# QWERTY6191/projected-lmc

Measured on AMD Instinct MI355X. Metric: MLL+grad iters/sec, n=8192 16-task LMC, higher is better.
Workload: dtype f32; 1 GPU; C3: ProjectedGPModel+ProjectedLMCmll exact training step (PLMC_fast), n=8192 d=8 p=16 q=8 Matern-5/2 fp32; latents sharded q/N per GPU; n_points=8192, n_dim=8, n_tasks=16, n_latents=8, parallelism=latent-shard x1

## Files before the change

### projected-lmc_amd/csrc/api.hip

```cpp
#include <stdlib.h>
#include <mutex>
#include <vector>

#include "api_common.hpp"
#include "../../include/plmc.h"

namespace plmc {
char *err_buf() {
  static thread_local char buf[256] = {0};
  return buf;
}

static const char *kProfNames[PK_COUNT] = {"k_assemble", "k_write_rhs", "k_assemble_cross", "k_diag",   "k_panel",
                                           "k_trail",    "k_wdiag",     "k_trtri_row",      "k_extract_col",
                                           "k_wt_matvec", "k_kinv_grad", "k_reduce_grad", "k_kernel_vjp",
                                           "sweep_total", "k_trail_row", "k_trail_head", "k_gpanel", "k_split_w", "k_posterior_moments", "k_trmm_ut"};
struct ProfRec { int id; hipEvent_t a, b; double flops, bytes; };
static unsigned g_prof_mask = 0;
static std::vector<ProfRec> g_recs;
static std::vector<hipEvent_t> g_free;

static hipEvent_t get_event() {
  if (!g_free.empty()) { hipEvent_t e = g_free.back(); g_free.pop_back(); return e; }
  hipEvent_t e;
  if (hipEventCreate(&e) != hipSuccess) return nullptr;
  return e;
}

static std::recursive_mutex g_api_mutex;
void api_lock() { g_api_mutex.lock(); }
void api_unlock() { g_api_mutex.unlock(); }

static Knobs g_knobs;
static bool g_knobs_loaded = false;
static void load_knobs() {
  const char *h = getenv("PLMC_HALF_TILES"), *g = getenv("PLMC_GRP");
  g_knobs.half_tiles = h ? (atoi(h) == 1 ? 1e30 : (double)atoi(h)) : 640.0;
  g_knobs.grp = g ? atoi(g) : 0;
  g_knobs.serial = getenv("PLMC_SERIAL") && atoi(getenv("PLMC_SERIAL")) != 0;
  g_knobs.bulk_lds = getenv("PLMC_BULK_LDS") ? atoi(getenv("PLMC_BULK_LDS")) : -1;
  g_knobs.split = getenv("PLMC_SPLIT") ? atoi(getenv("PLMC_SPLIT")) : 2;
  if (g_knobs.split != 0 && g_knobs.split != 3) g_knobs.split = 2;
  g_knobs.bulk_streams = getenv("PLMC_BULK_STREAMS") ? atoi(getenv("PLMC_BULK_STREAMS")) : 2;
  g_knobs.chain = getenv("PLMC_CHAIN") ? atoi(getenv("PLMC_CHAIN")) : 1;
  g_knobs.chain_nw = getenv("PLMC_CHAIN_NW") ? atoi(getenv("PLMC_CHAIN_NW")) : 0;
  g_knobs.chain_edge = getenv("PLMC_CHAIN_EDGE") ? atoi(getenv("PLMC_CHAIN_EDGE")) : 0;
  g_knobs_loaded = true;
}
const Knobs &knobs() {
  if (!g_knobs_loaded) {
    std::lock_guard<std::recursive_mutex> lk(g_api_mutex);
    if (!g_knobs_loaded) load_knobs();
  }
  return g_knobs;
}

constexpr int SWEEP_CTX = 2;
struct SweepCtx {
  hipStream_t caller = nullptr;
  bool used = false;
  unsigned long long stamp = 0;
  hipStream_t side[2] = {nullptr, nullptr};
  hipEvent_t ev[16] = {nullptr};
};
static SweepCtx g_ctx[64][SWEEP_CTX];
static unsigned long long g_stamp = 0;
static thread_local int t_ctx = 0;
static SweepCtx *cur_ctx() {
  int dev = 0;
  if (hipGetDevice(&dev) != hipSuccess || dev < 0 || dev >= 64) return nullptr;
  return &g_ctx[dev][t_ctx];
}
hipStream_t side_stream(int which) {
  SweepCtx *c = cur_ctx();
  if (!c || which < 0 || which > 1) return nullptr;
  if (!c->side[which]) {
    int lo = 0, hi = 0;
    (void)hipDeviceGetStreamPriorityRange(&lo, &hi);
    if (hipStreamCreateWithPriority(&c->side[which], hipStreamNonBlocking, hi) != hipSuccess) c->side[which] = nullptr;
  }
  return c->side[which];
}
hipEvent_t sync_event(int idx) {
  SweepCtx *c = cur_ctx();
  if (!c) return nullptr;
  hipEvent_t &e = c->ev[idx & 15];
  if (!e && hipEventCreateWithFlags(&e, hipEventDisableTiming) != hipSuccess) e = nullptr;
  return e;
}
void bind_sweep_ctx(hipStream_t caller, int e_prev_idx) {
  int dev = 0;
  if (hipGetDevice(&dev) != hipSuccess || dev < 0 || dev >= 64) { t_ctx = 0; return; }
  SweepCtx *set = g_ctx[dev];
  int pick = -1;
  for (int i = 0; i < SWEEP_CTX; ++i)
    if (set[i].used && set[i].caller == caller) pick = i;
  if (pick < 0) {
    for (int i = 0; i < SWEEP_CTX && pick < 0; ++i)
      if (!set[i].used) pick = i;
    if (pick < 0) {
      pick = 0;
      for (int i = 1; i < SWEEP_CTX; ++i)
        if (set[i].stamp < set[pick].stamp) pick = i;
      if (set[pick].ev[e_prev_idx & 15]) (void)hipStreamWaitEvent(caller, set[pick].ev[e_prev_idx & 15], 0);
    }
    set[pick].caller = caller;
    set[pick].used = true;
  }
  set[pick].stamp = ++g_stamp;
  t_ctx = pick;
}

template <typename T>
__global__ __launch_bounds__(NTHREADS) void k_mfma_rate(T *sink, int iters) {
  using Tr = Traits<T>;
  typename Tr::acc_t acc[16];
#pragma unroll
  for (int i = 0; i < 16; ++i)
#pragma unroll
    for (int r = 0; r < 4; ++r) acc[i][r] = T(0);
  T a[4], b[4];
#pragma unroll
  for (int i = 0; i < 4; ++i) { a[i] = T(1) + T(threadIdx.x & 7) * T(1e-3) + T(i); b[i] = T(0.5) - T(i) * T(1e-3); }
#pragma unroll 1
  for (int it = 0; it < iters; ++it) {
#pragma unroll
    for (int i = 0; i < 16; ++i) acc[i] = Tr::mfma(a[i >> 2], b[i & 3], acc[i]);
  }
  T s = T(0);
#pragma unroll
  for (int i = 0; i < 16; ++i) s += acc[i][0] + acc[i][1] + acc[i][2] + acc[i][3];
  sink[(size_t)blockIdx.x * NTHREADS + threadIdx.x] = s;
}

typedef __bf16 rate_bf16x8 __attribute__((ext_vector_type(8)));
__global__ __launch_bounds__(NTHREADS) void k_mfma_rate_bf16(float *sink, int iters) {
  f32x4 acc[16];
#pragma unroll
  for (int i = 0; i < 16; ++i)
#pragma unroll
    for (int r = 0; r < 4; ++r) acc[i][r] = 0.f;
  rate_bf16x8 a[4], b[4];
#pragma unroll
  for (int i = 0; i < 4; ++i)
#pragma unroll
    for (int j = 0; j < 8; ++j) { a[i][j] = (__bf16)(1.0f + 0.01f * (float)((threadIdx.x + j) & 7) + (float)i); b[i][j] = (__bf16)(0.5f - 0.01f * (float)(i + j)); }
#pragma unroll 1
  for (int it = 0; it < iters; ++it) {
#pragma unroll
    for (int i = 0; i < 16; ++i) acc[i] = __builtin_amdgcn_mfma_f32_16x16x32_bf16(a[i >> 2], b[i & 3], acc[i], 0, 0, 0);
  }
  float s = 0.f;
#pragma unroll
  for (int i = 0; i < 16; ++i) s += acc[i][0] + acc[i][1] + acc[i][2] + acc[i][3];
  sink[(size_t)blockIdx.x * NTHREADS + threadIdx.x] = s;
}

template <typename T, bool BF16 = false> static int mfma_rate_impl(void *sink, int64_t sink_bytes, double *tflops) {
  int dev = 0;
  hipDeviceProp_t prop;
  if (hipGetDevice(&dev) != hipSuccess || hipGetDeviceProperties(&prop, dev) != hipSuccess) return fail("plmc_prof_mfma_rate", "no device");
  const int grid = 4 * prop.multiProcessorCount, iters = 4000;
  if (!sink || !tflops || sink_bytes < (int64_t)grid * NTHREADS * (int64_t)sizeof(T)) return fail("plmc_prof_mfma_rate", "sink too small");
  hipEvent_t e0 = nullptr, e1 = nullptr;
  if (hipEventCreate(&e0) != hipSuccess || hipEventCreate(&e1) != hipSuccess) return fail("plmc_prof_mfma_rate", "event");
  double best = 0.0;
  for (int rep = 0; rep < 3; ++rep) {
    (void)hipEventRecord(e0, nullptr);
    if (BF16) hipLaunchKernelGGL(k_mfma_rate_bf16, dim3(grid), dim3(NTHREADS), 0, nullptr, (float *)sink, iters);
    else hipLaunchKernelGGL(k_mfma_rate<T>, dim3(grid), dim3(NTHREADS), 0, nullptr, (T *)sink, iters);
    (void)hipEventRecord(e1, nullptr);
    float ms = 0.f;
    if (hipEventSynchronize(e1) != hipSuccess || hipEventElapsedTime(&ms, e0, e1) != hipSuccess) break;
    const double fl = (double)grid * (NTHREADS / 64) * (double)iters * 16.0 * 2.0 * 16 * 16 * (BF16 ? 32 : 4);
    if (ms > 0.f && fl / (ms * 1e-3) / 1e12 > best) best = fl / (ms * 1e-3) / 1e12;
  }
  (void)hipEventDestroy(e0);
  (void)hipEventDestroy(e1);
  *tflops = best;
  return launch_status("plmc_prof_mfma_rate");
}

ProfScope::ProfScope(int id, hipStream_t st, double flops, double bytes) : idx_(-1), st_(st) {
  api_lock();
  if (!((g_prof_mask >> id) & 1u) || g_recs.size() >= (1u << 20)) return;
  ProfRec r{id, get_event(), get_event(), flops, bytes};
  if (!r.a || !r.b) return;
  (void)hipEventRecord(r.a, st);
  g_recs.push_back(r);
  idx_ = (long)g_recs.size() - 1;
}
ProfScope::~ProfScope() {
  if (idx_ >= 0) (void)hipEventRecord(g_recs[idx_].b, st_);
  api_unlock();
}
}

extern "C" {
// ... 40 lines not shown
```

### projected-lmc_amd/csrc/api_common.hpp

```cpp
#pragma once
#include <hip/hip_runtime.h>
#include <stdint.h>
#include <stdio.h>
#include <string.h>

#include "gemm_core.hpp"
#include "covariance.hpp"

namespace plmc {

constexpr int MAX_DIM = 32;
constexpr int MAX_COMP = 4;
constexpr int SM_MAX_MIX = 8;
constexpr int SM_MAX_DIM = 8;
constexpr int PER_MAX_DIM = 8;
constexpr int RQ_MAX_DIM = 16;
constexpr int LPER_MAX_DIM = 8;
constexpr int DOT_MAX_DIM = 16;
constexpr int DOT_MAX_POWER = 8;
constexpr int SUM_MAX_DIM = 8;
constexpr int FAM_PUBLIC_BASE = 16;
enum { F_PER = 5, F_RQ = 6, F_LPER = 7 };

char *err_buf();

inline int fail(const char *fn, const char *msg) {
  snprintf(err_buf(), 256, "%s: %s", fn, msg);
  return -1;
}

inline int launch_status(const char *fn) {
  hipError_t e = hipGetLastError();
  if (e != hipSuccess) {
    snprintf(err_buf(), 256, "%s: HIP launch failed: %s", fn, hipGetErrorString(e));
    return -2;
  }
  return 0;
}

#define PLMC_REQUIRE(cond, msg) \
  do { if (!(cond)) return plmc::fail(__func__, msg); } while (0)

enum ProfKernel { PK_ASSEMBLE, PK_WRITE_RHS, PK_CROSS, PK_DIAG, PK_PANEL, PK_TRAIL, PK_WDIAG, PK_TRTRI, PK_EXTRACT,
                  PK_WTMV, PK_KINV_GRAD, PK_REDUCE, PK_VJP, PK_SWEEP, PK_TRAIL_ROW, PK_TRAIL_HEAD, PK_GPANEL, PK_SPLIT, PK_POST, PK_TRMM, PK_COUNT };

struct ProfScope {
  ProfScope(int id, hipStream_t st, double flops, double bytes);
  ~ProfScope();
  long idx_;
  hipStream_t st_;
};

struct Knobs {
  double half_tiles;
  int grp;
  bool serial;
  int bulk_lds;
  int split;
  int bulk_streams;
  int chain;
  int chain_edge;
  int chain_nw;
};
const Knobs &knobs();

enum CovFamily { COV_PLAIN, COV_ADD, COV_SM, COV_PER, COV_RQ, COV_LPER, COV_SUM, COV_DOT };
struct CovTable {
  CovFamily family;
  int kind, d, ncomp;
  const void *ell, *second, *oscale;
  const void *third = nullptr;
  int fams = 0;
  bool of_sum = false;
  static CovTable plain(int kind, int d, const void *ell, const void *oscale) { return {COV_PLAIN, kind, d, 1, ell, nullptr, oscale}; }
  static CovTable add(int kind, int d, int ncomp, const void *ell, const void *oscale) { return {COV_ADD, kind, d, ncomp, ell, nullptr, oscale}; }
  static CovTable sm(int d, int nmix, const void *scales, const void *means, const void *weights) { return {COV_SM, 0, d, nmix, scales, means, weights}; }
  static CovTable per(int d, const void *ell, const void *period, const void *oscale) { return {COV_PER, 0, d, 1, ell, period, oscale}; }
  static CovTable rq(int d, const void *ell, const void *alpha, const void *oscale) { return {COV_RQ, 0, d, 1, ell, alpha, oscale}; }
  static CovTable lper(int d, const void *ell, const void *period, const void *rbf_ell, const void *oscale) {
    return {COV_LPER, 0, d, 1, ell, period, oscale, rbf_ell};
  }
  static CovTable dot(int d, int power, const void *v, const void *c, const void *oscale) { return {COV_DOT, 0, d, power, v, c, oscale}; }
  int power() const { return ncomp; }
  static CovTable sum(int d, int ncomp, const int *fam, const void *table, const void *oscale) {
    CovTable t{COV_SUM, 0, d, ncomp, table, nullptr, oscale};
    if (!fam) t.fams = -3;
    if (!fam || ncomp < 1 || ncomp > MAX_COMP) return t;
    for (int g = 0; g < ncomp; ++g) {
      const int f = fam[g];
      int code;
      if (f >= K_RBF && f <= K_MATERN52) code = f;
      else if (f >= FAM_PUBLIC_BASE && f <= FAM_PUBLIC_BASE + 2) code = F_PER + (f - FAM_PUBLIC_BASE);
      else { t.fams = f == K_SPLINE ? -2 : -1; return t; }
      t.fams |= code << (4 * g);
    }
    return t;
  }
  int fam_of(int g) const { return (fams >> (4 * g)) & 15; }
  CovTable member(const void *ell_, const void *period_, const void *rbf_, const void *alpha_, const void *os_) const {
    const int f = fam_of(0);
    CovTable t = f == F_PER ? per(d, ell_, period_, os_) : f == F_RQ ? rq(d, ell_, alpha_, os_) : f == F_LPER ? lper(d, ell_, period_, rbf_, os_)
                                                                                                          : plain(f, d, ell_, os_);
    t.of_sum = true;
    return t;
  }
  template <typename T> CovTable member_of_latent(int lat) const {
    const T *rec = (const T *)ell + (int64_t)lat * (3 * d + 1);
    return member(rec, rec + d, rec + 2 * d, rec + 3 * d, oscale ? (const T *)oscale + lat : nullptr);
  }
  bool single_member() const { return family == COV_SUM && ncomp == 1; }
  const char *check() const {
    if (family == COV_SUM) {
      if (ncomp < 1 || ncomp > MAX_COMP) return "need 1 <= components <= plmc_sum_max_components()";
      if (d <= 0 || d > SUM_MAX_DIM) return "need 0 < d <= plmc_sum_max_dim()";
      if (fams == -3 || !ell) return "null pointer";
      if (fams == -2) return "the spline kernel is not a member of a sum (members: the stationary kinds 0..3, PLMC_FAM_PERIODIC, PLMC_FAM_RQ, PLMC_FAM_LPER)";
      if (fams < 0) return "unknown member family code (members: the stationary kinds 0..3, PLMC_FAM_PERIODIC, PLMC_FAM_RQ, PLMC_FAM_LPER; no spectral mixture)";
      return nullptr;
    }
    if (family == COV_ADD) {
      if (kind < 0 || kind > K_MATERN52) return "additive kernels take the stationary kinds only (no spline kernel)";
      if (ncomp < 1 || ncomp > MAX_COMP) return "need 1 <= components <= plmc_max_components()";
    } else if (family == COV_SM) {
      if (ncomp < 1 || ncomp > SM_MAX_MIX) return "need 1 <= mixtures <= plmc_sm_max_mixtures()";
      if (d <= 0 || d > SM_MAX_DIM) return "need 0 < d <= plmc_sm_max_dim()";
    } else if (family == COV_PER) {
      if (d <= 0 || d > PER_MAX_DIM) return "need 0 < d <= plmc_per_max_dim()";
    } else if (family == COV_RQ) {
      if (d <= 0 || d > RQ_MAX_DIM) return "need 0 < d <= plmc_rq_max_dim()";
    } else if (family == COV_LPER) {
      if (d <= 0 || d > LPER_MAX_DIM) return "need 0 < d <= plmc_lper_max_dim()";
      if (!third) return "null pointer";
    } else if (family == COV_DOT) {
      if (d <= 0 || d > DOT_MAX_DIM) return "need 0 < d <= plmc_dot_max_dim()";
      if (ncomp < 1 || ncomp > DOT_MAX_POWER) return "need 1 <= power <= plmc_dot_max_power()";
    }
    return (family == COV_SM || family == COV_PER || family == COV_RQ || family == COV_LPER || family == COV_DOT) && !second ? "null pointer" : nullptr;
  }
  CovFamily route() const { return family == COV_ADD && ncomp == 1 ? COV_PLAIN : family; }
  int partials_rows() const { return family == COV_ADD || family == COV_SM || family == COV_SUM ? ncomp : 1; }
};
#define PLMC_REQUIRE_TABLE(t) \
  do { if (const char *why_ = (t).check()) return plmc::fail(__func__, why_); } while (0)

struct AssembleJob {
  CovTable table;
  int n;
  const void *X, *noise;
};
int assemble_rows(const AssembleJob &job, int elem_bytes, void *A, int64_t lda, int64_t strideA, int q, int ib0, int nrows, void *stream,
                  int ncols = -1, int skip = 0);

hipStream_t side_stream(int which = 0);
hipEvent_t sync_event(int idx);
void bind_sweep_ctx(hipStream_t caller, int e_prev_idx);

inline bool aligned16(const void *p) { return (reinterpret_cast<uintptr_t>(p) & 15) == 0; }

}
```

### projected-lmc_amd/csrc/potrf.hip

```cpp
#include <stdlib.h>
#include "api_common.hpp"
#include "covariance.hpp"
#include "diag_block.hpp"
#include "bf3_engine.hpp"
#include "chain_engine.hpp"
#include "vd_layout.hpp"
#include "../../include/plmc.h"

namespace plmc {

template <typename T> constexpr int CHAIN_BURST = sizeof(T) == 8 ? 4 : 8;

template <typename T> struct ColMap {
  int u0, nU, Taug, w0, nW;
  int64_t n_pad;
  T *W;
  int64_t ldw, strideW;
};

template <typename T, int NT, bool BURSTED = false>
__global__ __launch_bounds__(NTHREADS, TILE_MIN_WAVES<T>) void k_panel(T *A, int64_t lda, int64_t strideA, int r, ColMap<T> cm,
                                                     const T *__restrict__ Vd, int64_t strideV) {
  __builtin_amdgcn_s_setprio(3);
  __shared__ __align__(16) T smem[tile_smem_elems<T>()];
// ... 513 lines not shown
  else if (t < cm.nU + cm.Taug) { colp = cm.n_pad + (int64_t)(t - cm.nU) * NB; D = A + (int64_t)lat * strideA + (int64_t)g0 * NB * lda + colp; }
  else {
    ldd = cm.ldw;
    colp = wcol0 + (int64_t)(cm.w0 + t - cm.nU - cm.Taug) * NB;
    D = cm.W + (int64_t)lat * cm.strideW + (int64_t)g0 * NB * ldd + (int64_t)(cm.w0 + t - cm.nU - cm.Taug) * NB;
  }
  const int nm = (G + 1) / 2;
  const unsigned short *Vp = VgP + (int64_t)lat * vgp_lat_stride, *Rp = Praw + (int64_t)lat * praw_lat_stride + colp * 8;
  unsigned short *Pp = Pl + (int64_t)lat * pl_lat_stride + colp * 8;
  int64_t pld = lda;
  if (fam == 1) { Pp = Wk + (int64_t)lat * wk_lat_stride + b3_index<S>((int64_t)g0 * NB, 0, colp - wcol0, cm.n_pad); pld = cm.n_pad; }
  const int half = __builtin_amdgcn_readfirstlane((int)threadIdx.x >> 8), tid = (int)threadIdx.x & 255;
#pragma unroll 1
  for (int pass = 0; pass < 2; ++pass) {
    const int a = pass == 0 ? nm - 1 - y : ((paired && y < nm - 1 - y) ? y : -1);
    if (a < 0) break;
    const int i0 = 2 * a, rows = G - i0 < 2 ? G - i0 : 2;
    Acc<float> acc0, acc1;
    acc0.zero();
    acc1.zero();
    b3_mainloop<S>(acc0, acc1, Vp + (int64_t)i0 * NB * 8, (int64_t)GMAX * NB, Rp, lda, (i0 + rows) * NB, lds);
    b3_combine<S>(acc0, acc1, unscale);
    const int i = i0 + half;
    b3_writeback<S, WB_STORE, true>(acc0, D + (int64_t)i * NB * ldd, ldd, reinterpret_cast<float *>(lds + half * B3_WB_BYTES), tid, half < rows,
                                    Pp + (int64_t)i * 16 * S::NPL * pld * 8, pld, true, pscale);
    __syncthreads();
  }
}

template <typename T>
__global__ __launch_bounds__(NTHREADS) void k_extract_col(const T *__restrict__ A, int64_t n_pad, int64_t lda,
                                                           int64_t strideA, int c, T *__restrict__ z,
                                                           double *__restrict__ quad) {
  __shared__ double red[NTHREADS];
  const int lat = blockIdx.x;
  const T *Al = A + (int64_t)lat * strideA + n_pad + c;
  double s = 0.0;
  for (int64_t i = threadIdx.x; i < n_pad; i += NTHREADS) {
    T v = Al[i * lda];
    z[(int64_t)lat * n_pad + i] = v;
    s += (double)v * (double)v;
  }
  red[threadIdx.x] = s;
  __syncthreads();
  for (int o = NTHREADS / 2; o > 0; o >>= 1) {
    if (threadIdx.x < o) red[threadIdx.x] += red[threadIdx.x + o];
    __syncthreads();
  }
  if (threadIdx.x == 0) quad[lat] = red[0];
}

constexpr int WTMV_NT = 1024;
template <typename T, int CW = NB>
__global__ __launch_bounds__(WTMV_NT * CW / NB) void k_wt_matvec(const T *__restrict__ W, int64_t n_pad, int64_t ldw,
                                                                 int64_t strideW, const T *__restrict__ z,
                                                                 T *__restrict__ alpha) {
  using vec_t = typename Traits<T>::vec_t;
  constexpr int EPV = Traits<T>::EPV;
  constexpr int LPR = CW / EPV;
  constexpr int NRG = WTMV_NT / (NB / EPV);
  __shared__ double red[NRG][CW];
  const int lat = blockIdx.y;
  const int cl = (threadIdx.x % LPR) * EPV, rg = threadIdx.x / LPR;
  const int64_t colw = (int64_t)blockIdx.x * CW;
  const int64_t col0 = colw / NB * NB;
  const T *Wl = W + (int64_t)lat * strideW + colw + cl;
  const T *zl = z + (int64_t)lat * n_pad;
  double s[EPV];
#pragma unroll
  for (int e = 0; e < EPV; ++e) s[e] = 0.0;
  constexpr int U = CW == NB ? 4 : 8;
  for (int64_t l = col0 + rg; l < n_pad; l += U * NRG) {
    vec_t v[U];
    T zz[U];
#pragma unroll
    for (int u = 0; u < U; ++u) {
      const int64_t ll = l + u * NRG;
      const int64_t lc = ll < n_pad ? ll : n_pad - 1;
      v[u] = *reinterpret_cast<const vec_t *>(Wl + lc * ldw);
      const T zv = zl[lc];
      zz[u] = ll < n_pad ? zv : T(0);
    }
#pragma unroll
    for (int u = 0; u < U; ++u)
#pragma unroll
      for (int e = 0; e < EPV; ++e) s[e] += (double)v[u][e] * (double)zz[u];
  }
#pragma unroll
  for (int e = 0; e < EPV; ++e) red[rg][cl + e] = s[e];
  __syncthreads();
  if (threadIdx.x < CW) {
    double t = 0.0;
#pragma unroll
    for (int g = 0; g < NRG; ++g) t += red[g][threadIdx.x];
    alpha[(int64_t)lat * n_pad + colw + threadIdx.x] = (T)t;
  }
}

template <typename T>
__global__ __launch_bounds__(WTMV_NT) void k_w_diag(const T *__restrict__ W, int64_t n_pad, int64_t ldw, int64_t strideW,
                                                    T *__restrict__ kd) {
  using vec_t = typename Traits<T>::vec_t;
  constexpr int EPV = Traits<T>::EPV;
  constexpr int LPR = 128 / EPV;
  constexpr int NRG = WTMV_NT / LPR;
  __shared__ double red[NRG][NB];
  const int lat = blockIdx.y;
  const int cl = (threadIdx.x % LPR) * EPV, rg = threadIdx.x / LPR;
  const int64_t col0 = (int64_t)blockIdx.x * NB;
  const T *Wl = W + (int64_t)lat * strideW + col0 + cl;
  double s[EPV];
#pragma unroll
  for (int e = 0; e < EPV; ++e) s[e] = 0.0;
  for (int64_t l = col0 + rg; l < n_pad; l += 4 * NRG) {
    vec_t v[4];
#pragma unroll
    for (int u = 0; u < 4; ++u) {
      const int64_t ll = l + u * NRG;
      v[u] = *reinterpret_cast<const vec_t *>(Wl + (ll < n_pad ? ll : n_pad - 1) * ldw);
    }
#pragma unroll
    for (int u = 0; u < 4; ++u)
      if (l + u * NRG < n_pad) {
#pragma unroll
        for (int e = 0; e < EPV; ++e) s[e] += (double)v[u][e] * (double)v[u][e];
      }
  }
#pragma unroll
  for (int e = 0; e < EPV; ++e) red[rg][cl + e] = s[e];
  __syncthreads();
  if (threadIdx.x < NB) {
    double t = 0.0;
#pragma unroll
    for (int g = 0; g < NRG; ++g) t += red[g][threadIdx.x];
    kd[(int64_t)lat * n_pad + col0 + threadIdx.x] = (T)t;
  }
}

template <typename T, class S>
struct Sweep {
  static constexpr bool bf3 = !std::is_void<S>::value;
  static_assert(!bf3 || sizeof(T) == 4, "split schemes stand in for fp32 products");
  static constexpr double nb = NB, nb3 = nb * nb * nb, esz = sizeof(T);

  T *A;
  int64_t n_pad, lda, strideA, naug_pad, wcol0;
  int q, m, Taug;
  bool with_inverse, keep;
  const float *eig_lo = nullptr;
  double *logdet = nullptr;
  int *info = nullptr;
  T *Vd, *Wg, *Vg2[2], *Ph, *Pbulk;
  unsigned short *Pl[2], *Praw, *VgP2[2], *Wk, *Uk;
  float *scl;
  int64_t strideV, pl_lat, sc_lat, uk_step;
  T *WA;
  const Knobs &kn;
  double hthr;
  unsigned bulk_lds;
  int grp, ng, chain_pool;
  hipStream_t st, C = nullptr, H = nullptr;
  hipEvent_t e_entry = nullptr, e_v = nullptr, e_gh = nullptr, e_p = nullptr, e_hd = nullptr, e_tail = nullptr, e_doneC = nullptr,
             e_doneH = nullptr, e_prev = nullptr, e_sc = nullptr;

  Sweep(T *A_, int64_t n_pad_, int64_t lda_, int naug, int64_t wcol0_, int64_t strideA_, T *Vd_, int q_, bool with_inverse_, bool keep_,
        int grp_, unsigned bulk_lds_, hipStream_t st_)
      : A(A_), n_pad(n_pad_), lda(lda_), strideA(strideA_), naug_pad(plmc_pad(naug)), wcol0(wcol0_), q(q_), m((int)(n_pad_ / NB)),
        Taug((int)(plmc_pad(naug) / NB)), with_inverse(with_inverse_), keep(keep_), Vd(Vd_), kn(knobs()), hthr(kn.half_tiles),
        bulk_lds(bulk_lds_), grp(grp_), st(st_) {
    const VdLayout L(n_pad, lda, (int)sizeof(T), keep);
    strideV = L.stride();
    pl_lat = L.stride_u16();
    sc_lat = L.stride_f32();
    Wg = L.at<T>(Vd, L.wg);
    Ph = L.at<T>(Vd, L.ph);
    Pbulk = L.at<T>(Vd, L.pbulk);
    for (int b = 0; b < 2; ++b) {
      Vg2[b] = L.at<T>(Vd, L.vg[b]);
      Pl[b] = bf3 ? L.at<unsigned short>(Vd, L.pl[b]) : nullptr;
      VgP2[b] = bf3 ? L.at<unsigned short>(Vd, L.vgp[b]) : nullptr;
    }
    Praw = bf3 ? L.at<unsigned short>(Vd, L.praw) : nullptr;
    scl = bf3 ? L.at<float>(Vd, L.scl) : nullptr;
    Wk = (bf3 && with_inverse) ? L.at<unsigned short>(Vd, L.wk) : nullptr;
    Uk = keep ? L.at<unsigned short>(Vd, L.uk) : nullptr;
    uk_step = L.plane_blocks * NB * NB * 2;
    WA = with_inverse ? A + wcol0 : nullptr;
    ng = (m + grp - 1) / grp;
    chain_pool = kn.chain_nw > 0 ? (kn.chain_nw < 200 ? kn.chain_nw : 200) : (q >= 8 ? 80 : (q >= 4 ? 44 : (q >= 2 ? 36 : 31)));
  }

  int G0(int gi) const { return gi < ng ? gi * grp : m; }
  ColMap<T> cm_tri(int g0, int u0, int nU, int w0, int nW) const {
    return ColMap<T>{u0, nU, 0, w0, nW, n_pad, Wg - (int64_t)g0 * NB * LDG - (int64_t)g0 * NB, (int64_t)LDG, strideV};
  }
  ColMap<T> cm_buf(int u0, int nU, int taug, int w0, int nW) const { return ColMap<T>{u0, nU, taug, w0, WA ? nW : 0, n_pad, WA, lda, strideA}; }
  unsigned short *planes(int g0) const { return keep ? Uk + (int64_t)(g0 / grp) * uk_step : Pl[(g0 / grp) & 1]; }

  void clear() {
    hipLaunchKernelGGL(k_zero_diag_out<T>, dim3(m > GMAX ? m : GMAX, q), dim3(NTHREADS), 0, st, Vd, strideV, m, Wg, (int64_t)LDG,
                       strideV, (int64_t)NB * LDG + NB, GMAX, VdLayout::CTR);
  }
  void diag(int r, int g0, hipStream_t s) {
    ProfScope ps(PK_DIAG, s, q * (2.0 / 3.0) * nb3, q * 3.0 * nb * nb * esz);
    T *wout = Wg + (int64_t)(r - g0) * NB * LDG + (int64_t)(r - g0) * NB;
    hipLaunchKernelGGL((k_diag<T>), dim3(q), dim3(DIAG_NT), 0, s, A, lda, strideA, r, Vd, strideV, wout, (int64_t)LDG, strideV);
  }
  void panel(int r, const ColMap<T> &cm, hipStream_t s) {
    const int nt = cm.nU + cm.Taug + cm.nW;
    if (nt == 0) return;
    ProfScope ps(PK_PANEL, s, q * (double)nt * nb3, q * 2.0 * nt * nb * nb * esz);
    if ((double)nt * q <= hthr && q <= 2)
      hipLaunchKernelGGL((k_panel<T, 2, true>), dim3(nt, q, 2), dim3(NTHREADS), 0, s, A, lda, strideA, r, cm, Vd, strideV);
    else if ((double)nt * q <= hthr)
      hipLaunchKernelGGL((k_panel<T, 2>), dim3(nt, q, 2), dim3(NTHREADS), 0, s, A, lda, strideA, r, cm, Vd, strideV);
    else
      hipLaunchKernelGGL((k_panel<T, 4>), dim3(nt, q, 1), dim3(NTHREADS), 0, s, A, lda, strideA, r, cm, Vd, strideV);
  }
  void update(int ib0, int nrows, int r_lo, int r_hi, const ColMap<T> &cm, hipStream_t s, int cls, int skip_ib = 0, int skip_jb = 0,
              bool crit = false, int raw_end = 0) {
    const int Cn = cm.nU + cm.Taug + cm.nW;
    if (nrows <= 0 || Cn == 0) return;
    const double depth = (r_hi - r_lo + 1) * nb, nr = (double)nrows;
    double tilesU = 0.0, halfU = 0.0;
    for (int i = 0; i < nrows; ++i)
      for (int t = 0; t < cm.nU; ++t) {
        const int ib = ib0 + i, jb = cm.u0 + t;
        if (jb < ib || (ib < skip_ib && jb < skip_jb)) continue;
        tilesU += 1.0;
        if (jb == ib) halfU += 0.5;
      }
    double depthW = 0.0;
    int nfirst = 0;
    for (int c = 0; c < cm.nW; ++c) {
      const int cb = cm.w0 + c;
      depthW += (cb >= r_lo ? (r_hi - cb + 1) : (r_hi - r_lo + 1)) * nb;
      nfirst += cb >= r_lo;
    }
    const double flops = 2.0 * nb * nb * (depth * (tilesU - halfU) + nr * (depth * cm.Taug + depthW));
    const double bytes = (2.0 * (tilesU + nr * (cm.Taug + cm.nW)) - nr * nfirst) * nb * nb * esz;
    ProfScope ps(cls, s, q * flops, q * bytes);
    if constexpr (bf3) {
      if (cls == PK_TRAIL || cls == PK_TRAIL_HEAD) {
        const dim3 grid(Cn, (nrows + 1) / 2, q);
        const unsigned short *pl = planes(r_lo);
#define PLMC_UPD3(ROLE)                                                                                                                    \
  hipLaunchKernelGGL((k_update_bf3<S, ROLE>), grid, dim3(B3_NT), 0, s, A, lda, strideA, ib0, nrows, r_lo, r_hi, cm, skip_ib, skip_jb, pl, \
                     pl_lat, wcol0, Praw, pl_lat, raw_end, (const float *)scl, sc_lat, Wk, pl_lat)
        if (cls == PK_TRAIL) PLMC_UPD3(0);
        else if (crit) PLMC_UPD3(2);
        else PLMC_UPD3(3);
#undef PLMC_UPD3
        return;
      }
    }
    const bool half = cls != PK_TRAIL && (double)Cn * nrows * q <= hthr;
    const unsigned dyn = (cls == PK_TRAIL || (cls == PK_TRAIL_HEAD && !crit)) ? bulk_lds : 0u;
    const dim3 grid(Cn, half ? 2 * nrows : nrows, q);
#define PLMC_UPD(ROLE, MT) \
  hipLaunchKernelGGL((k_update<T, ROLE, MT>), grid, dim3(NTHREADS), dyn, s, A, lda, strideA, ib0, r_lo, r_hi, cm, skip_ib, skip_jb)
    if (cls == PK_TRAIL_ROW) { if (half && q <= 2 && r_hi == r_lo) PLMC_UPD(4, 2); else if (half) PLMC_UPD(1, 2); else PLMC_UPD(1, 4); }
    else if (cls == PK_TRAIL_HEAD && crit) { if (half) PLMC_UPD(2, 2); else PLMC_UPD(2, 4); }
    else if (cls == PK_TRAIL_HEAD) { if (half) PLMC_UPD(3, 2); else PLMC_UPD(3, 4); }
    else PLMC_UPD(0, 4);
#undef PLMC_UPD
  }
  void gpanel(int g0, int G, const ColMap<T> &cm, int buf, hipStream_t s, int head) {
    const int nt = cm.nU + cm.Taug + cm.nW;
    if (nt == 0) return;
    const double prods = G * (G + 1) / 2.0;
    ProfScope ps(PK_GPANEL, s, q * (double)nt * prods * 2.0 * nb3, q * (double)nt * (prods + G) * nb * nb * esz);
    if constexpr (bf3) {
      const int nm = (G + 1) / 2;
      hipLaunchKernelGGL((k_gpanel_bf3<S>), dim3(nt, head ? nm : (nm + 1) / 2, q), dim3(B3_NT), 0, s, A, lda, strideA, g0, G, cm,
                         (const unsigned short *)VgP2[buf], pl_lat, (const unsigned short *)Praw, pl_lat, planes(g0), pl_lat, wcol0,
                         (const float *)scl, sc_lat, head ? 0 : 1, Wk, pl_lat);
    } else {
      T *Pb = head ? Ph : Pbulk;
      const int64_t ldp = head ? (int64_t)LDG : lda;
      if (head)
        hipLaunchKernelGGL((k_gpanel_rows<T, 1>), dim3(nt, 2 * G, q), dim3(NTHREADS), 0, s, (const T *)A, lda, strideA, g0, G, cm,
                           (const T *)Vg2[buf], (int64_t)LDG, strideV, Pb, ldp, strideV);
      else
        hipLaunchKernelGGL((k_gpanel_rows<T, 0>), dim3(nt, (G + 1) / 2, q), dim3(NTHREADS), bulk_lds, s, (const T *)A, lda, strideA, g0, G, cm,
                           (const T *)Vg2[buf], (int64_t)LDG, strideV, Pb, ldp, strideV);
      hipLaunchKernelGGL((k_gpanel_copy<T>), dim3(nt, G, q), dim3(NTHREADS), 0, s, A, lda, strideA, g0, cm, (const T *)Pb, ldp, strideV);
    }
  }
  void scan(hipStream_t s, int64_t row0, int64_t row1, int part0, int parts) {
    if constexpr (bf3) {
      if (S::NPL == 2)
        hipLaunchKernelGGL(k_scale_scan, dim3(parts, q), dim3(NTHREADS), 0, s, (const float *)A, n_pad, row0, row1, lda, strideA, (int)naug_pad, scl,
                           sc_lat, part0);
    }
  }
  void split_scales(hipStream_t s) {
    if constexpr (bf3) hipLaunchKernelGGL((k_split_scales<S>), dim3(q), dim3(64), 0, s, n_pad, eig_lo, scl, sc_lat);
  }
  int finish(hipStream_t s) {
    hipLaunchKernelGGL(k_logdet<T>, dim3(q), dim3(NTHREADS), 0, s, (const T *)A, n_pad, lda, strideA, logdet, info,
                       (const T *)(Wg + VdLayout::CTL), strideV, q);
    return launch_status("potrf_impl");
  }

  static constexpr int CHAIN_QB = 32;
  void chain(int gi, hipStream_t s) {
    const int g0 = G0(gi), g1 = G0(gi + 1);
    if (kn.chain) {
      const int G = g1 - g0;
      ProfScope ps(PK_DIAG, s, q * (2.0 / 3.0) * nb3 * G, q * 3.0 * nb * nb * esz * G);
      const bool edge = gi == 0 || gi + 2 >= ng;
      const int pool = (edge && kn.chain_edge > 0) ? kn.chain_edge : chain_pool;
      for (int l0 = 0; l0 < q; l0 += CHAIN_QB) {
        const int ql = q - l0 < CHAIN_QB ? q - l0 : CHAIN_QB;
        hipLaunchKernelGGL((k_chain<T>), dim3(ql + (G > 1 ? pool : 0)), dim3(CH_NT), 0, s, A + (int64_t)l0 * strideA, lda, strideA, g0, G,
                           Vd + (int64_t)l0 * strideV, strideV, Wg + (int64_t)l0 * strideV, strideV, ql);
      }
      return;
    }
    for (int r = g0; r < g1; ++r) {
      diag(r, g0, s);
      panel(r, cm_tri(g0, r + 1, g1 - 1 - r, g0, r - g0), s);
      if (r + 1 < g1) update(r + 1, g1 - r - 1, r, r, cm_tri(g0, r + 1, g1 - r - 1, g0, r + 1 - g0), s, PK_TRAIL_ROW);
    }
  }
  void vtrans(int gi, hipStream_t s, bool from_w = false) {
    const int g0 = G0(gi), G = G0(gi + 1) - g0;
    T *const tri = WA ? WA + (int64_t)g0 * NB * lda + (int64_t)g0 * NB : (T *)nullptr;
    hipLaunchKernelGGL((k_vtrans<T, S>), dim3(bf3 ? GMAX * GMAX : G * (G + 1) / 2, q), dim3(NTHREADS), 0, s, from_w ? (const T *)tri : (const T *)Wg,
                       from_w ? lda : (int64_t)LDG, from_w ? strideA : strideV, strideV, Vg2[gi & 1], G, from_w ? (T *)nullptr : tri, lda, strideA,
                       VgP2[gi & 1], pl_lat, (const float *)scl, sc_lat);
  }
  void wtri_planes(int gi, hipStream_t s) {
    if constexpr (bf3) {
      if (!WA) return;
      const int g0 = G0(gi), G = G0(gi + 1) - g0;
      hipLaunchKernelGGL((k_wtri_planes<S>), dim3(G * (G + 1) / 2, q), dim3(NTHREADS), 0, s, (const float *)WA, lda, strideA, g0, (const float *)scl,
                         sc_lat, Wk, pl_lat, n_pad);
    }
  }
  void raw_planes0(hipStream_t s, const ColMap<T> &cm) {
    if constexpr (bf3) {
      const int nt = cm.nU + cm.Taug + cm.nW;
      if (nt > 0)
        hipLaunchKernelGGL((k_raw_planes<S>), dim3(nt, G0(1), q), dim3(NTHREADS), 0, s, (const float *)A, lda, strideA, 0, cm, Praw, pl_lat, wcol0,
                           (const float *)scl, sc_lat);
    }
  }

  bool bind_streams() {
    if (!kn.serial) bind_sweep_ctx(st, 8);
    C = kn.serial ? nullptr : side_stream();
    H = kn.serial ? nullptr : (kn.bulk_streams == 1 ? st : side_stream(1));
    hipEvent_t *const ev[] = {&e_entry, &e_v, &e_gh, &e_p, &e_hd, &e_tail, &e_doneC, &e_doneH, &e_prev};
    bool la = C && H && ng > 2;
    for (int i = 0; i < 9; ++i) la = (*ev[i] = sync_event(i)) && la;
    e_sc = sync_event(12);
    return la;
  }

  int inputs(const AssembleJob *job) {
    if (job) {
      const int rc = assemble_rows(*job, (int)sizeof(T), A, lda, strideA, q, 0, m, st);
      if (rc != 0) return rc;
    }
    scan(st, 0, n_pad, 0, SCAN_PARTS);
    split_scales(st);
    return 0;
  }

  int one_stream(const AssembleJob *job) {
    const int rc = inputs(job);
    if (rc != 0) return rc;
    raw_planes0(st, cm_buf(G0(1), m - G0(1), Taug, 0, 0));
    for (int gi = 0; gi < ng; ++gi) {
      const int g0 = G0(gi), g1 = G0(gi + 1), g2 = G0(gi + 2);
      chain(gi, st);
      vtrans(gi, st);
      wtri_planes(gi, st);
      if (bf3) {
        gpanel(g0, g1 - g0, cm_buf(g1, g2 - g1, 0, 0, 0), gi & 1, st, 1);
        gpanel(g0, g1 - g0, cm_buf(g2, m - g2, Taug, 0, g0), gi & 1, st, 0);
        update(g1, m - g1, g0, g1 - 1, cm_buf(g1, m - g1, Taug, 0, g1), st, PK_TRAIL, g2, g2, false, g2);
        update(g1, g2 - g1, g0, g1 - 1, cm_buf(g1, g2 - g1, 0, 0, 0), st, PK_TRAIL_HEAD, 0, 0, true);
      } else {
        gpanel(g0, g1 - g0, cm_buf(g1, m - g1, Taug, 0, g0), gi & 1, st, 0);
        update(g1, m - g1, g0, g1 - 1, cm_buf(g1, m - g1, Taug, 0, g1), st, PK_TRAIL);
      }
    }
    return finish(st);
  }

  int lookahead(const AssembleJob *job) {
    const bool fused = job && e_sc;
    if (fused) {
      const int rc = assemble_rows(*job, (int)sizeof(T), A, lda, strideA, q, 0, G0(1), st, G0(1));
      if (rc != 0) return rc;
      scan(st, 0, (int64_t)G0(1) * NB, 0, SCAN_PARTS / 2);
    } else {
      const int rc = inputs(job);
      if (rc != 0) return rc;
    }
    (void)hipEventRecord(e_entry, st);
    (void)hipStreamWaitEvent(C, e_entry, 0);
    (void)hipStreamWaitEvent(H, e_entry, 0);
    if (fused) {
      const int rc = assemble_rows(*job, (int)sizeof(T), A, lda, strideA, q, 0, m, H, -1, G0(1));
      if (rc != 0) return rc;
      scan(H, (int64_t)G0(1) * NB, n_pad, SCAN_PARTS / 2, SCAN_PARTS / 2);
      split_scales(H);
      (void)hipEventRecord(e_sc, H);
    }
    raw_planes0(H, cm_buf(G0(1), m - G0(1), Taug, 0, 0));
    (void)hipEventRecord(e_hd, H);
    for (int gi = 0; gi < ng; ++gi) {
      const int g0 = G0(gi), g1 = G0(gi + 1), g2 = G0(gi + 2), G = g1 - g0;
      chain(gi, C);
      if (fused && gi == 0) (void)hipStreamWaitEvent(C, e_sc, 0);
      vtrans(gi, C);
      (void)hipEventRecord(e_v, C);
      if (gi > 0 || bf3) (void)hipStreamWaitEvent(C, e_hd, 0);
      gpanel(g0, G, cm_buf(g1, g2 - g1, 0, 0, 0), gi & 1, C, 1);
      (void)hipEventRecord(e_gh, C);
      if (gi > 0) (void)hipStreamWaitEvent(C, e_tail, 0);
      update(g1, g2 - g1, g0, g1 - 1, cm_buf(g1, g2 - g1, 0, 0, 0), C, PK_TRAIL_HEAD, 0, 0, true);

      (void)hipStreamWaitEvent(H, e_v, 0);
      wtri_planes(gi, H);
      gpanel(g0, G, cm_buf(g2, m - g2, Taug, 0, g0), gi & 1, H, 0);
      (void)hipEventRecord(e_p, H);
      (void)hipStreamWaitEvent(H, e_gh, 0);
      if (gi > 0) (void)hipStreamWaitEvent(H, e_tail, 0);
      update(g1, g2 - g1, g0, g1 - 1, cm_buf(g2, m - g2, Taug, 0, g1), H, PK_TRAIL_HEAD, 0, 0, false, g2);
      (void)hipEventRecord(e_hd, H);

      (void)hipStreamWaitEvent(st, e_p, 0);
      (void)hipStreamWaitEvent(st, e_gh, 0);
      update(g2, m - g2, g0, g1 - 1, cm_buf(g2, m - g2, Taug, 0, g1), st, PK_TRAIL);
      (void)hipEventRecord(e_tail, st);
    }
    const int rc_fin = finish(C);
    (void)hipEventRecord(e_doneC, C);
    (void)hipEventRecord(e_doneH, H);
    (void)hipStreamWaitEvent(st, e_doneC, 0);
    (void)hipStreamWaitEvent(st, e_doneH, 0);
    (void)hipEventRecord(e_prev, st);
    return rc_fin;
  }
};

template <typename T, class S>
int potrf_impl(T *A, int64_t n_pad, int64_t lda, int naug, int64_t strideA, T *Vd, double *logdet, int *info,
               int with_inverse_arg, int q, const float *eig_lo, void *stream, const AssembleJob *job = nullptr) {
  PLMC_REQUIRE((with_inverse_arg & 2) == 0, "with_inverse bit 1 (K^-1 accumulated in the sweep) is gone: use plmc_kinv_grad_* behind the sweep");
  const bool with_inverse = (with_inverse_arg & 1) != 0;
  const bool keep = !std::is_void<S>::value && (with_inverse_arg & 4) != 0 && with_inverse;
  PLMC_REQUIRE(A && Vd && logdet && info, "null pointer");
  PLMC_REQUIRE(n_pad > 0 && n_pad % NB == 0 && lda % NB == 0 && lda >= n_pad, "n_pad/lda must be multiples of NB");
  const int64_t naug_pad = plmc_pad(naug);
  PLMC_REQUIRE(naug >= 0 && n_pad + naug_pad + (with_inverse ? n_pad : 0) <= lda,
               "lda too small for naug (+ the n_pad columns of the inverse factor)");
  PLMC_REQUIRE(q > 0 && aligned16(A) && aligned16(Vd), "bad q or unaligned buffer");
  const Knobs &kn = knobs();
  const int grp = (!keep && kn.grp > 0 && kn.grp < GMAX) ? kn.grp : GMAX;
  const unsigned bulk_lds = (unsigned)(kn.bulk_lds >= 0 ? kn.bulk_lds : (q == 1 ? 20000 : (q == 2 ? 16000 : 0)));
  Sweep<T, S> sw(A, n_pad, lda, naug, n_pad + naug_pad, strideA, Vd, q, with_inverse, keep, grp, bulk_lds, (hipStream_t)stream);
  sw.eig_lo = eig_lo;
  sw.logdet = logdet;
  sw.info = info;
  const double npd = (double)n_pad;
  ProfScope whole(PK_SWEEP, sw.st, q * (with_inverse ? 2.0 : 1.0) * npd * npd * npd / 3.0, 0.0);
  sw.clear();
  return sw.bind_streams() ? sw.lookahead(job) : sw.one_stream(job);
}

bool vd_w_planes(const float *Vd, int64_t n_pad, int64_t lda, const unsigned short **wk, int64_t *wk_lat_stride, const float **w_scale,
                 int64_t *w_scale_lat_stride) {
  const VdLayout L(n_pad, lda, 4, false);
  if (L.wk < 0) return false;
  *wk = L.at<const unsigned short>(Vd, L.wk);
  *wk_lat_stride = L.stride_u16();
  *w_scale = L.at<const float>(Vd, L.scl) + SC_SW;
  *w_scale_lat_stride = L.stride_f32();
  return true;
}

template <typename T>
int potrs_aug_at(T *A, int64_t n_pad, int64_t lda, int naug, int64_t wcol0, int64_t strideA, T *Vd, int q, void *stream) {
  PLMC_REQUIRE(A && Vd, "null pointer");
  PLMC_REQUIRE(n_pad > 0 && n_pad % NB == 0 && lda % NB == 0 && wcol0 % NB == 0, "n_pad / lda / wcol0 must be multiples of NB");
  const int64_t naug_pad = plmc_pad(naug);
  PLMC_REQUIRE(naug > 0 && q > 0 && n_pad + naug_pad <= wcol0 && wcol0 + n_pad <= lda, "augmented columns must fit between the square part and the W columns");
  PLMC_REQUIRE(aligned16(A) && aligned16(Vd), "unaligned buffer");
  Sweep<T, void> sw(A, n_pad, lda, naug, wcol0, strideA, Vd, q, true, false, GMAX, 0u, (hipStream_t)stream);
  const ColMap<T> cm{0, 0, sw.Taug, 0, 0, n_pad, (T *)nullptr, lda, strideA};
  for (int gi = 0; gi < sw.ng; ++gi) {
    const int g0 = sw.G0(gi), g1 = sw.G0(gi + 1), G = g1 - g0;
    hipLaunchKernelGGL((k_vtrans<T, void>), dim3(G * (G + 1) / 2, q), dim3(NTHREADS), 0, sw.st, (const T *)(sw.WA + (int64_t)g0 * NB * lda + (int64_t)g0 * NB),
                       lda, strideA, sw.strideV, sw.Vg2[0], G, (T *)nullptr, lda, strideA, (unsigned short *)nullptr, (int64_t)0, (const float *)nullptr, (int64_t)0);
    sw.gpanel(g0, G, cm, 0, sw.st, 0);
    sw.update(g1, sw.m - g1, g0, g1 - 1, cm, sw.st, PK_TRAIL);
  }
  return launch_status("plmc_potrs_aug");
}

template <class S>
__global__ __launch_bounds__(64) void k_aug_scales(int64_t n_pad, float *__restrict__ sc, int64_t sc_stride) {
  if constexpr (S::NPL == 3) return;
  if (threadIdx.x != 0) return;
  float *o = sc + (int64_t)blockIdx.x * sc_stride;
  float amax = 0.0f;
  for (int p = 0; p < SCAN_PARTS; ++p) amax = fmaxf(amax, o[SC_N + 3 * p + 2]);
  const float D = o[6], lam = o[7];
  const float Rn = sqrtf((float)n_pad) * amax + 1e-30f;
  o[SC_SA] = b3_scale_for(Rn / sqrtf(lam));
  o[SC_RA] = b3_scale_for(Rn * (1.0f + sqrtf(D / lam)));
}

template <class S>
int potrs_aug_kept(float *A, int64_t n_pad, int64_t lda, int naug, int64_t wcol0, int64_t strideA, float *Vd, int q, void *stream) {
  PLMC_REQUIRE(A && Vd, "null pointer");
  PLMC_REQUIRE(n_pad > 0 && n_pad % NB == 0 && lda % NB == 0 && wcol0 % NB == 0, "n_pad / lda / wcol0 must be multiples of NB");
  const int64_t naug_pad = plmc_pad(naug);
  PLMC_REQUIRE(naug > 0 && q > 0 && n_pad + naug_pad <= wcol0 && wcol0 + n_pad <= lda, "augmented columns must fit between the square part and the W columns");
  PLMC_REQUIRE(aligned16(A) && aligned16(Vd), "unaligned buffer");
  Sweep<float, S> sw(A, n_pad, lda, naug, wcol0, strideA, Vd, q, true, true, GMAX, 0u, (hipStream_t)stream);
  const ColMap<float> cm{0, 0, sw.Taug, 0, 0, n_pad, (float *)nullptr, lda, strideA};
  hipLaunchKernelGGL(k_scale_scan, dim3(SCAN_PARTS, q), dim3(NTHREADS), 0, sw.st, (const float *)A, n_pad, (int64_t)0, n_pad, lda, strideA, (int)naug_pad,
                     sw.scl, sw.sc_lat, 0);
  hipLaunchKernelGGL((k_aug_scales<S>), dim3(q), dim3(64), 0, sw.st, n_pad, sw.scl, sw.sc_lat);
  sw.raw_planes0(sw.st, cm);
  for (int gi = 0; gi < sw.ng; ++gi) {
    const int g0 = sw.G0(gi), g1 = sw.G0(gi + 1);
    sw.vtrans(gi, sw.st, true);
    sw.gpanel(g0, g1 - g0, cm, gi & 1, sw.st, 0);
    sw.update(g1, sw.m - g1, g0, g1 - 1, cm, sw.st, PK_TRAIL, 0, 0, false, sw.G0(gi + 2));
  }
  return launch_status("plmc_potrs_aug_kept");
}

template <typename T>
int extract_col_impl(const T *A, int64_t n_pad, int64_t lda, int64_t strideA, int c, T *z, double *quad, int q,
                     void *stream) {
  PLMC_REQUIRE(A && z && quad, "null pointer");
  PLMC_REQUIRE(c >= 0 && n_pad + c < lda, "column outside the augmented block");
  ProfScope ps(PK_EXTRACT, (hipStream_t)stream, 0.0, q * 2.0 * n_pad * sizeof(T));
  hipLaunchKernelGGL(k_extract_col<T>, dim3(q), dim3(NTHREADS), 0, (hipStream_t)stream, A, n_pad, lda, strideA, c, z,
                     quad);
  return launch_status(__func__);
}

template <typename T>
int wt_matvec_impl(const T *W, int64_t n_pad, int64_t ldw, int64_t strideW, const T *z, T *alpha, int q,
                   void *stream) {
  PLMC_REQUIRE(W && z && alpha, "null pointer");
  PLMC_REQUIRE(n_pad > 0 && n_pad % NB == 0, "n_pad must be a multiple of NB");
  ProfScope ps(PK_WTMV, (hipStream_t)stream, q * (double)n_pad * n_pad, q * ((double)n_pad * n_pad / 2) * sizeof(T));
  if ((int64_t)q * (n_pad / NB) < 128)
    hipLaunchKernelGGL((k_wt_matvec<T, 32>), dim3((unsigned)(n_pad / 32), q), dim3(WTMV_NT / 4), 0, (hipStream_t)stream, W, n_pad, ldw, strideW, z,
                       alpha);
  else
    hipLaunchKernelGGL((k_wt_matvec<T, NB>), dim3((unsigned)(n_pad / NB), q), dim3(WTMV_NT), 0, (hipStream_t)stream, W, n_pad, ldw, strideW, z,
                       alpha);
  return launch_status(__func__);
}

template <typename T>
int w_diag_impl(const T *W, int64_t n_pad, int64_t ldw, int64_t strideW, T *kinv_diag, int q, void *stream) {
  PLMC_REQUIRE(W && kinv_diag, "null pointer");
  PLMC_REQUIRE(n_pad > 0 && n_pad % NB == 0 && q > 0 && aligned16(W), "n_pad must be a multiple of NB");
  ProfScope ps(PK_WTMV, (hipStream_t)stream, q * (double)n_pad * n_pad, q * ((double)n_pad * n_pad / 2) * sizeof(T));
  hipLaunchKernelGGL(k_w_diag<T>, dim3((unsigned)(n_pad / NB), q), dim3(WTMV_NT), 0, (hipStream_t)stream, W, n_pad, ldw, strideW,
                     kinv_diag);
  return launch_status(__func__);
}

}

extern "C" {
int64_t plmc_vd_blocks_for(int64_t n_pad, int64_t lda, int elem_bytes) { return plmc::VdLayout(n_pad, lda, elem_bytes, false).blocks; }
int64_t plmc_vd_blocks(int64_t n_pad, int64_t lda) { return plmc_vd_blocks_for(n_pad, lda, 4); }
int64_t plmc_vd_blocks_keep(int64_t n_pad, int64_t lda) { return plmc::VdLayout(n_pad, lda, 4, true).blocks; }
int64_t plmc_split_scales_offset(int64_t n_pad, int64_t lda) { return plmc::VdLayout(n_pad, lda, 4, false).scl * plmc::NB * plmc::NB; }
static int potrf_f32_any(float *A, int64_t n_pad, int64_t lda, int naug, int64_t strideA, float *Vd, double *logdet, int *info,
                         int with_inverse, int q, const float *eig_lo, void *stream, const plmc::AssembleJob *job = nullptr) {
  const int split = plmc::knobs().split;
  if (split == 0) return plmc::potrf_impl<float, void>(A, n_pad, lda, naug, strideA, Vd, logdet, info, with_inverse, q, nullptr, stream, job);
  if (split == 2 && eig_lo)
    return plmc::potrf_impl<float, plmc::SplitH2>(A, n_pad, lda, naug, strideA, Vd, logdet, info, with_inverse, q, eig_lo, stream, job);
  return plmc::potrf_impl<float, plmc::SplitB3>(A, n_pad, lda, naug, strideA, Vd, logdet, info, with_inverse, q, nullptr, stream, job);
}
int plmc_factorize_ex_f32(int kind, const float *X, int n, int d, const float *ell, const float *oscale, const float *noise, float *A,
// ... 192 lines not shown
```

### projected-lmc_amd/csrc/vd_layout.hpp

```cpp
#pragma once
#include <stdint.h>

#include "gemm_core.hpp"

namespace plmc {

constexpr int GMAX = 8;
constexpr int LDG = (GMAX + 1) * NB;
constexpr int VD_FIXED_BLOCKS = 4 * GMAX * (GMAX + 1);

enum { SC_SU = 0, SC_SW = 1, SC_RU = 2, SC_RW = 3, SC_SA = 4, SC_RA = 5, SC_N = 8, SC_TAG = 8 + 3 * 32 };
constexpr int SCAN_PARTS = 32;
constexpr int VD_W_TAG = SC_TAG - SC_SW;

inline int64_t vd_wk_blocks(int64_t n_pad, int64_t lda, int elem_bytes) {
  const int64_t m = n_pad / NB;
  return (elem_bytes == 4 && lda >= 2 * n_pad) ? (3 * m * m + 1) / 2 : 0;
}

struct VdLayout {
  static constexpr int64_t CTR = (int64_t)GMAX * NB, CTL = LDG + (int64_t)GMAX * NB;

  int elem_bytes;
  int64_t wg, vg[2], ph, pbulk;
  int64_t pl[2] = {-1, -1}, praw = -1, vgp[2] = {-1, -1}, scl = -1, wk = -1, uk = -1;
  int64_t plane_blocks = 0;
  int64_t blocks;

  VdLayout(int64_t n_pad, int64_t lda, int elem_bytes_, bool keep) : elem_bytes(elem_bytes_) {
    const int64_t m = n_pad / NB, ldb = (lda + NB - 1) / NB, grp = GMAX * (GMAX + 1);
    wg = m;
    vg[0] = wg + grp;
    vg[1] = vg[0] + grp;
    ph = vg[1] + grp;
    pbulk = ph + grp;
    int64_t b = pbulk + GMAX * ldb;
    if (elem_bytes == 4) {
      plane_blocks = 3 * GMAX * ldb / 2;
      const int64_t vgp_blocks = 6 * GMAX * GMAX / 4;
      pl[0] = b;
      pl[1] = pl[0] + plane_blocks;
      praw = pl[1] + plane_blocks;
      vgp[0] = praw + plane_blocks;
      vgp[1] = vgp[0] + vgp_blocks;
      scl = vgp[1] + vgp_blocks;
      b = scl + 1;
      if (vd_wk_blocks(n_pad, lda, 4) > 0) {
        wk = b;
        b += vd_wk_blocks(n_pad, lda, 4);
      }
      if (keep) {
        uk = b;
        b += ((m + GMAX - 1) / GMAX) * plane_blocks;
      }
    }
    blocks = b;
  }
  int64_t stride() const { return blocks * NB * NB; }
  int64_t stride_u16() const { return stride() * (elem_bytes / 2); }
  int64_t stride_f32() const { return stride() * elem_bytes / 4; }
  template <class U, class V> U *at(V *Vd, int64_t blk) const {
    return blk < 0 ? nullptr : reinterpret_cast<U *>(Vd + blk * (int64_t)NB * NB);
  }
};

bool vd_w_planes(const float *Vd, int64_t n_pad, int64_t lda, const unsigned short **wk, int64_t *wk_lat_stride, const float **w_scale,
                 int64_t *w_scale_lat_stride);

}
```

Baseline: 60.69 iters/sec.

## Split blocked Cholesky trailing update into near/far parts with paired group tails

Adds a tail-pair mode, on by default, for the bf3 blocked Cholesky sweep. The trailing update for each panel group becomes a near update that covers only the next group and uses a new kernel role, plus a far update of the rest that runs only on every second group and accumulates two panel groups at once. The far update reads from four rotating plane slots carved out of the pbulk/pl region instead of two. This shortens the critical path to the next panel (the tail event is recorded after the near part) and halves the launches over the large far trailing region, at the cost of more buffer slots and correctness hinging on the slot aliasing and the pairing bookkeeping.

```diff
diff --git a/projected-lmc_amd/csrc/api.hip b/projected-lmc_amd/csrc/api.hip
--- a/projected-lmc_amd/csrc/api.hip
+++ b/projected-lmc_amd/csrc/api.hip
@@ -44,6 +44,7 @@
   g_knobs.bulk_streams = getenv("PLMC_BULK_STREAMS") ? atoi(getenv("PLMC_BULK_STREAMS")) : 2;
   g_knobs.chain = getenv("PLMC_CHAIN") ? atoi(getenv("PLMC_CHAIN")) : 1;
   g_knobs.chain_nw = getenv("PLMC_CHAIN_NW") ? atoi(getenv("PLMC_CHAIN_NW")) : 0;
+  g_knobs.tail_pair = getenv("PLMC_TAIL_PAIR") ? atoi(getenv("PLMC_TAIL_PAIR")) : 1;
   g_knobs.chain_edge = getenv("PLMC_CHAIN_EDGE") ? atoi(getenv("PLMC_CHAIN_EDGE")) : 0;
   g_knobs_loaded = true;
 }
diff --git a/projected-lmc_amd/csrc/api_common.hpp b/projected-lmc_amd/csrc/api_common.hpp
--- a/projected-lmc_amd/csrc/api_common.hpp
+++ b/projected-lmc_amd/csrc/api_common.hpp
@@ -60,6 +60,7 @@
   int bulk_streams;
   int chain;
   int chain_edge;
+  int tail_pair;
   int chain_nw;
 };
 const Knobs &knobs();
diff --git a/projected-lmc_amd/csrc/potrf.hip b/projected-lmc_amd/csrc/potrf.hip
--- a/projected-lmc_amd/csrc/potrf.hip
+++ b/projected-lmc_amd/csrc/potrf.hip
@@ -689,8 +689,11 @@
   int *info = nullptr;
   T *Vd, *Wg, *Vg2[2], *Ph, *Pbulk;
   unsigned short *Pl[2], *Praw, *VgP2[2], *Wk, *Uk;
+  unsigned short *Pl4 = nullptr;
   float *scl;
   int64_t strideV, pl_lat, sc_lat, uk_step;
+  int64_t slot_step = 0;
+  bool pair = false;
   T *WA;
   const Knobs &kn;
   double hthr;
@@ -724,6 +727,11 @@
     uk_step = L.plane_blocks * NB * NB * 2;
     WA = with_inverse ? A + wcol0 : nullptr;
     ng = (m + grp - 1) / grp;
+    if constexpr (bf3) {
+      slot_step = b3_elems<S>((int64_t)grp * NB, lda);
+      pair = kn.tail_pair != 0 && !keep && 4 * slot_step <= L.slot_room();
+      if (pair) Pl4 = L.at<unsigned short>(Vd, L.pbulk);
+    }
     chain_pool = kn.chain_nw > 0 ? (kn.chain_nw < 200 ? kn.chain_nw : 200) : (q >= 8 ? 80 : (q >= 4 ? 44 : (q >= 2 ? 36 : 31)));
   }
 
@@ -732,7 +740,11 @@
     return ColMap<T>{u0, nU, 0, w0, nW, n_pad, Wg - (int64_t)g0 * NB * LDG - (int64_t)g0 * NB, (int64_t)LDG, strideV};
   }
   ColMap<T> cm_buf(int u0, int nU, int taug, int w0, int nW) const { return ColMap<T>{u0, nU, taug, w0, WA ? nW : 0, n_pad, WA, lda, strideA}; }
-  unsigned short *planes(int g0) const { return keep ? Uk + (int64_t)(g0 / grp) * uk_step : Pl[(g0 / grp) & 1]; }
+  unsigned short *planes(int g0) const {
+    const int gi = g0 / grp;
+    return keep ? Uk + (int64_t)gi * uk_step : (pair ? Pl4 + (int64_t)(gi & 3) * slot_step : Pl[gi & 1]);
+  }
+  int pair_lo(int gi) const { return G0((gi & 1) ? gi - 1 : gi); }
 
   void clear() {
     hipLaunchKernelGGL(k_zero_diag_out<T>, dim3(m > GMAX ? m : GMAX, q), dim3(NTHREADS), 0, st, Vd, strideV, m, Wg, (int64_t)LDG,
@@ -755,7 +767,7 @@
       hipLaunchKernelGGL((k_panel<T, 4>), dim3(nt, q, 1), dim3(NTHREADS), 0, s, A, lda, strideA, r, cm, Vd, strideV);
   }
   void update(int ib0, int nrows, int r_lo, int r_hi, const ColMap<T> &cm, hipStream_t s, int cls, int skip_ib = 0, int skip_jb = 0,
-              bool crit = false, int raw_end = 0) {
+              bool crit = false, int raw_end = 0, bool near = false) {
     const int Cn = cm.nU + cm.Taug + cm.nW;
     if (nrows <= 0 || Cn == 0) return;
     const double depth = (r_hi - r_lo + 1) * nb, nr = (double)nrows;
@@ -784,7 +796,8 @@
 #define PLMC_UPD3(ROLE)                                                                                                                    \
   hipLaunchKernelGGL((k_update_bf3<S, ROLE>), grid, dim3(B3_NT), 0, s, A, lda, strideA, ib0, nrows, r_lo, r_hi, cm, skip_ib, skip_jb, pl, \
                      pl_lat, wcol0, Praw, pl_lat, raw_end, (const float *)scl, sc_lat, Wk, pl_lat)
-        if (cls == PK_TRAIL) PLMC_UPD3(0);
+        if (cls == PK_TRAIL && near) PLMC_UPD3(1);
+        else if (cls == PK_TRAIL) PLMC_UPD3(0);
         else if (crit) PLMC_UPD3(2);
         else PLMC_UPD3(3);
 #undef PLMC_UPD3
@@ -885,6 +898,16 @@
     }
   }
 
+  void near(int gi, hipStream_t s) {
+    const int g1 = G0(gi + 1), g2 = G0(gi + 2), g3 = G0(gi + 3);
+    update(g2, g3 - g2, pair_lo(gi), g1 - 1, cm_buf(g2, m - g2, Taug, 0, g1), s, PK_TRAIL, 0, 0, false, 0, true);
+  }
+  void far(int gi, hipStream_t s) {
+    if (!(gi & 1)) return;
+    const int g1 = G0(gi + 1), g3 = G0(gi + 3);
+    update(g3, m - g3, pair_lo(gi), g1 - 1, cm_buf(g3, m - g3, Taug, 0, g1), s, PK_TRAIL);
+  }
+
   bool bind_streams() {
     if (!kn.serial) bind_sweep_ctx(st, 8);
     C = kn.serial ? nullptr : side_stream();
@@ -918,7 +941,13 @@
       if (bf3) {
         gpanel(g0, g1 - g0, cm_buf(g1, g2 - g1, 0, 0, 0), gi & 1, st, 1);
         gpanel(g0, g1 - g0, cm_buf(g2, m - g2, Taug, 0, g0), gi & 1, st, 0);
-        update(g1, m - g1, g0, g1 - 1, cm_buf(g1, m - g1, Taug, 0, g1), st, PK_TRAIL, g2, g2, false, g2);
+        if (pair) {
+          update(g1, g2 - g1, g0, g1 - 1, cm_buf(g2, m - g2, Taug, 0, g1), st, PK_TRAIL_HEAD, 0, 0, false, g2);
+          near(gi, st);
+          far(gi, st);
+        } else {
+          update(g1, m - g1, g0, g1 - 1, cm_buf(g1, m - g1, Taug, 0, g1), st, PK_TRAIL, g2, g2, false, g2);
+        }
         update(g1, g2 - g1, g0, g1 - 1, cm_buf(g1, g2 - g1, 0, 0, 0), st, PK_TRAIL_HEAD, 0, 0, true);
       } else {
         gpanel(g0, g1 - g0, cm_buf(g1, m - g1, Taug, 0, g0), gi & 1, st, 0);
@@ -973,8 +1002,14 @@
 
       (void)hipStreamWaitEvent(st, e_p, 0);
       (void)hipStreamWaitEvent(st, e_gh, 0);
-      update(g2, m - g2, g0, g1 - 1, cm_buf(g2, m - g2, Taug, 0, g1), st, PK_TRAIL);
-      (void)hipEventRecord(e_tail, st);
+      if (pair) {
+        near(gi, st);
+        (void)hipEventRecord(e_tail, st);
+        far(gi, st);
+      } else {
+        update(g2, m - g2, g0, g1 - 1, cm_buf(g2, m - g2, Taug, 0, g1), st, PK_TRAIL);
+        (void)hipEventRecord(e_tail, st);
+      }
     }
     const int rc_fin = finish(C);
     (void)hipEventRecord(e_doneC, C);
diff --git a/projected-lmc_amd/csrc/vd_layout.hpp b/projected-lmc_amd/csrc/vd_layout.hpp
--- a/projected-lmc_amd/csrc/vd_layout.hpp
+++ b/projected-lmc_amd/csrc/vd_layout.hpp
@@ -56,6 +56,7 @@
     }
     blocks = b;
   }
+  int64_t slot_room() const { return praw < 0 ? 0 : (praw - pbulk) * (int64_t)NB * NB * 2; }
   int64_t stride() const { return blocks * NB * NB; }
   int64_t stride_u16() const { return stride() * (elem_bytes / 2); }
   int64_t stride_f32() const { return stride() * elem_bytes / 4; }
```

Measured after the change: 61.70 iters/sec, median of 6. +1.7%, better.
